# DHDev0/Stochastic-muzero

Measured on AMD Instinct MI355X. Metric: MCTS simulations/sec (whole node), CartPole MLP 4096 envs × 50 sims, higher is better.
Workload: dtype f32 (tree values, heads) + f64 (pUCT scores, root priors) + i32 (counts)

## Files before the change

### include/smz.h

```cpp
#ifndef SMZ_H
#define SMZ_H

#include <stddef.h>
#include <stdint.h>

#ifdef __cplusplus
extern "C" {
#endif

#define SMZ_ABI_VERSION 1
#define SMZ_MAX_ACTIONS 32
#define SMZ_MAX_ACTIONS_LARGE 1024
#define SMZ_MAX_PLAYER_CYCLE 32
#define SMZ_MT_WORDS 624

typedef enum {
    SMZ_OK = 0,
    SMZ_ERR_INVALID = -1,
    SMZ_ERR_HIP = -2,
    SMZ_ERR_NOMEM = -3,
    SMZ_ERR_STATE = -4,
    SMZ_ERR_TOO_LARGE = -5
} smz_status;

// ... 65 lines not shown

int smz_expand_backup_select(smz_handle *h, const float *hidden_dev, const float *reward_dev, const float *policy_dev,
                             const float *value_dev, float *parent_hidden_dev, int32_t *last_action_dev,
                             uint8_t *branch_dev, float *mlp_input_dev, smz_stream stream);

int smz_root_stats(smz_handle *h, int32_t *visits_dev, double *priors_dev, float *root_value_dev,
                   float *child_reward_dev, smz_stream stream);

int smz_act(smz_handle *h, double temperature, const double *pow_table_host, int32_t *action_dev, double *policy_dev,
            double *child_visits_dev, float *root_value_dev, smz_stream stream);

int smz_support_decode(const float *logits_dev, int S, float *out_dev, int B, smz_stream stream);
int smz_policy_softmax(const float *logits_dev, int A, float *out_dev, int B, smz_stream stream);
int smz_dynamics_epilogue(const float *state_dyn_dev, const float *state_after_dev, const float *reward_logits_dev,
                          int ld, const uint8_t *branch_dev, int S, float *hidden_out_dev, float *reward_out_dev, int B,
                          smz_stream stream);
int smz_prediction_epilogue(const float *policy_logits_pred_dev, const float *value_logits_pred_dev,
                            const float *policy_logits_after_dev, const float *value_logits_after_dev, int ld,
                            const uint8_t *branch_dev, int A, int S, float *policy_out_dev, float *value_out_dev,
                            int B, smz_stream stream);

typedef struct {
    int32_t obs, A, S, H, L;
    int32_t OP;
    int32_t total_floats;
    int32_t off[30];
} smz_mlp_desc;
int smz_mlp_layout(smz_mlp_desc *desc);
int smz_mlp_initial(const smz_mlp_desc *desc, const float *weights_dev, const float *obs_dev, float *hidden_out_dev,
                    float *policy_out_dev, int B, smz_stream stream);
int smz_mlp_recurrent(const smz_mlp_desc *desc, const float *weights_dev, const float *mlp_input_dev,
                      const uint8_t *branch_dev, float *hidden_out_dev, float *reward_out_dev, float *policy_out_dev,
                      float *value_out_dev, int B, smz_stream stream);

enum { SMZ_LSTM_TRUNKS = 7, SMZ_LSTM_MAX_LAYERS = 4, SMZ_LSTM_REP = 2 * SMZ_LSTM_TRUNKS * SMZ_LSTM_MAX_LAYERS,
       SMZ_LSTM_OFFSETS = SMZ_LSTM_REP + 2, SMZ_LSTM_SLACK = 256 };
typedef struct {
    int32_t obs, A, S, L;
    int32_t total_floats;
    int32_t recurrent_floats;
    int32_t lds_bytes;
    int32_t off[SMZ_LSTM_OFFSETS];
} smz_lstm_desc;
int smz_lstm_layout(smz_lstm_desc *desc);
int smz_lstm_initial(const smz_lstm_desc *desc, const float *weights_dev, const float *obs_dev, float *hidden_out_dev,
                     float *policy_out_dev, int B, smz_stream stream);
int smz_lstm_recurrent(const smz_lstm_desc *desc, const float *weights_dev, const float *mlp_input_dev,
                       const uint8_t *branch_dev, float *hidden_out_dev, float *reward_out_dev, float *policy_out_dev,
                       float *value_out_dev, int B, smz_stream stream);

enum { SMZ_V_DYN = 0, SMZ_V_ADY = 1, SMZ_V_PRE = 2, SMZ_V_APR = 3 };
enum { SMZ_VT_CONV_IN = 0, SMZ_VT_BN_IN, SMZ_VT_RES_A, SMZ_VT_RES_B, SMZ_VT_RES_BN, SMZ_VT_MIX_W, SMZ_VT_MIX_B,
       SMZ_VT_TOWER , SMZ_V_TRANS_STRIDE = 13 };
enum { SMZ_VP_RES_A = 0, SMZ_VP_RES_B, SMZ_VP_RES_BN, SMZ_VP_VMIX_W, SMZ_VP_VMIX_B, SMZ_VP_VTOWER ,
       SMZ_VP_PMIX_W = 11, SMZ_VP_PMIX_B, SMZ_VP_PTOWER , SMZ_V_PRED_STRIDE = 19 };
enum { SMZ_VR_STEM = 0, SMZ_VR_NARROW_A, SMZ_VR_NARROW_B, SMZ_VR_NARROW_BN, SMZ_VR_WIDEN, SMZ_VR_WIDE_A, SMZ_VR_WIDE_B,
       SMZ_VR_WIDE_BN, SMZ_VR_LAST_A, SMZ_VR_LAST_B, SMZ_VR_LAST_BN };
enum { SMZ_V_TRANS_BASE = 0, SMZ_V_PRED_BASE = 26, SMZ_V_REP_BASE = 64, SMZ_V_OFFSETS = 80 };
typedef struct smz_vision_desc {
    int32_t A, S, H, L;
    int32_t OP;
    int32_t total_floats;
    int32_t small_floats;
    int32_t off[SMZ_V_OFFSETS];
} smz_vision_desc;
int smz_vision_layout(smz_vision_desc *desc);
// ... 104 lines not shown
```

### stochastic-muzero_amd/_lib.py

```python
import ctypes as C
import os

_HERE = os.path.dirname(os.path.abspath(__file__))
LIB_PATH = os.environ.get("SMZ_LIB_PATH") or os.path.join(_HERE, "libsmz.so")

SMZ_OK, SMZ_ERR_INVALID, SMZ_ERR_HIP, SMZ_ERR_NOMEM, SMZ_ERR_STATE, SMZ_ERR_TOO_LARGE = 0, -1, -2, -3, -4, -5
RNG_MT19937_NUMPY, RNG_PHILOX = 0, 1
MAX_ACTIONS = 32
MAX_ACTIONS_LARGE = 1024


class SmzError(RuntimeError):
    def __init__(self, code, text):
        super().__init__(f"libsmz error {code}: {text}")
        self.code = code


class Config(C.Structure):
    _fields_ = [("num_trees", C.c_int32), ("num_actions", C.c_int32), ("max_action_sample", C.c_int32),
                ("hidden_size", C.c_int32), ("num_simulations", C.c_int32), ("pb_c_base", C.c_int32),
                ("pb_c_init", C.c_double), ("discount", C.c_double), ("root_dirichlet_alpha", C.c_double),
                ("root_exploration_fraction", C.c_double), ("rng_mode", C.c_int32), ("device", C.c_int32)]


# ... 30 lines not shown


_P = C.c_void_p
SIGNATURES = {
    "smz_create": (C.c_int, [C.POINTER(Config), C.POINTER(_P)]),
    "smz_create_large_actions": (C.c_int, [C.POINTER(Config), C.POINTER(_P)]),
    "smz_destroy": (C.c_int, [_P]),
    "smz_abi_version": (C.c_int, []),
    "smz_build_features": (C.c_int, []),
    "smz_last_error": (C.c_char_p, []),
    "smz_node_capacity": (C.c_int, [_P]),
    "smz_last_kernel": (C.c_int, [_P, C.c_char_p, C.c_int]),
    "smz_set_pb_c_table": (C.c_int, [_P, _P, C.c_int]),
    "smz_seed": (C.c_int, [_P, _P, _P]),
    "smz_set_rng_state": (C.c_int, [_P, C.c_int, _P, C.c_int]),
    "smz_get_rng_state": (C.c_int, [_P, C.c_int, _P, C.POINTER(C.c_int)]),
    "smz_philox_words": (C.c_int, [C.c_uint64, C.c_uint32, C.c_int, C.c_int, _P]),
    "smz_get_philox_position": (C.c_int, [_P, C.c_int, C.POINTER(C.c_uint32), C.POINTER(C.c_int)]),
    "smz_rng_snapshot": (C.c_int, [_P, _P]),
    "smz_rng_restore": (C.c_int, [_P, _P]),
    "smz_root_init": (C.c_int, [_P, _P, _P, _P, C.c_int, _P]),
    "smz_select": (C.c_int, [_P, _P, _P, _P, _P, _P]),
    "smz_expand_backup": (C.c_int, [_P, _P, _P, _P, _P, _P]),
    "smz_expand_backup_select": (C.c_int, [_P, _P, _P, _P, _P, _P, _P, _P, _P, _P]),
    "smz_root_stats": (C.c_int, [_P, _P, _P, _P, _P, _P]),
    "smz_act": (C.c_int, [_P, C.c_double, _P, _P, _P, _P, _P, _P]),
    "smz_support_decode": (C.c_int, [_P, C.c_int, _P, C.c_int, _P]),
    "smz_policy_softmax": (C.c_int, [_P, C.c_int, _P, C.c_int, _P]),
    "smz_dynamics_epilogue": (C.c_int, [_P, _P, _P, C.c_int, _P, C.c_int, _P, _P, C.c_int, _P]),
    "smz_prediction_epilogue": (C.c_int, [_P, _P, _P, _P, C.c_int, _P, C.c_int, C.c_int, _P, _P, C.c_int, _P]),
    "smz_mlp_layout": (C.c_int, [C.POINTER(MlpDesc)]),
    "smz_mlp_initial": (C.c_int, [C.POINTER(MlpDesc), _P, _P, _P, _P, C.c_int, _P]),
    "smz_mlp_recurrent": (C.c_int, [C.POINTER(MlpDesc), _P, _P, _P, _P, _P, _P, _P, C.c_int, _P]),
    "smz_mlp_layout_wide": (C.c_int, [C.POINTER(MlpDesc)]),
    "smz_mlp_recurrent_wide": (C.c_int, [C.POINTER(MlpDesc), _P, _P, _P, _P, _P, _P, _P, C.c_int, _P]),
    "smz_lstm_layout": (C.c_int, [C.POINTER(LstmDesc)]),
    "smz_lstm_initial": (C.c_int, [C.POINTER(LstmDesc), _P, _P, _P, _P, C.c_int, _P]),
    "smz_lstm_recurrent": (C.c_int, [C.POINTER(LstmDesc), _P, _P, _P, _P, _P, _P, _P, C.c_int, _P]),
    "smz_vision_layout": (C.c_int, [C.POINTER(VisionDesc)]),
    "smz_vision_initial": (C.c_int, [C.POINTER(VisionDesc), _P, _P, _P, _P, C.c_int, _P]),
    "smz_vision_initial_record": (C.c_int, [C.POINTER(VisionDesc), _P, _P, _P, _P, _P, C.c_int, _P]),
    "smz_vision_recurrent": (C.c_int, [C.POINTER(VisionDesc), _P, _P, C.c_int, _P, _P, _P, _P, _P, _P, C.c_int, _P]),
    "smz_search_mlp_act": (C.c_int, [_P, C.POINTER(MlpDesc), _P, _P, C.c_int, C.c_double, _P, _P, _P, _P, _P, _P]),
    "smz_search_mlp_act_cartpole": (C.c_int, [_P, C.POINTER(MlpDesc), _P, C.c_int, C.c_double, _P, _P, _P, _P, _P,
                                              C.POINTER(CartPoleEnv), _P]),
    "smz_search_mlp": (C.c_int, [_P, C.POINTER(MlpDesc), _P, _P, C.c_int, _P]),
    "smz_frames_resize_u8": (C.c_int, [_P, C.c_int, C.c_int, C.c_int, C.c_int, C.c_int, _P, _P, _P]),
    "smz_frames_resize_taps_u8": (C.c_int, [_P, C.c_int, C.c_int, C.c_int, C.c_int, C.c_int, _P, _P, _P]),
    "smz_host_register": (C.c_int, [_P, C.c_size_t]),
    "smz_host_unregister": (C.c_int, [_P]),
    "smz_copy_async": (C.c_int, [_P, _P, C.c_size_t, C.c_int, _P]),
    "smz_search_vision": (C.c_int, [_P, C.POINTER(VisionDesc), _P, _P, _P, C.c_int, _P]),
    "smz_search_vision_act": (C.c_int, [_P, C.POINTER(VisionDesc), _P, _P, _P, C.c_int, C.c_double, _P, _P, _P, _P, _P, _P]),
    "smz_cartpole_step": (C.c_int, [_P, _P, _P, _P, _P, C.c_int, _P]),
    "smz_cartpole_step_pack": (C.c_int, [_P, _P, _P, _P, _P, _P, C.c_int, C.c_int, _P, _P, _P, C.c_int, _P]),
    "smz_cartpole_step_ctl": (C.c_int, [_P, _P, _P, _P, _P, C.POINTER(EpisodeCtl), _P, C.c_int, C.c_int, _P, _P, _P, C.c_int, _P]),
    "smz_cartpole_reset_state": (C.c_int, [C.c_uint64, C.c_int64, C.c_int64, C.POINTER(C.c_double * 4)]),
    "smz_synthetic_obs": (C.c_int, [_P, C.c_int, C.c_int, C.c_uint64, C.c_int64, C.c_int64, _P]),
    "smz_set_active": (C.c_int, [_P, _P]),
    "smz_set_players": (C.c_int, [_P, C.c_int, _P, _P]),
    "smz_set_leaf_ids_out": (C.c_int, [_P, _P]),
    "smz_host_cartpole_step": (C.c_int, [_P, _P, _P, _P, _P, _P, C.c_int32, C.c_int]),
    "smz_get_hidden_layout": (C.c_int, [_P, C.POINTER(_P), C.POINTER(C.c_int), C.POINTER(C.c_int)]),
    "smz_mlp_recurrent_rows": (C.c_int, [C.POINTER(MlpDesc), _P, _P, C.c_int, C.c_int, _P, _P, _P, _P, _P, _P, C.c_int, _P]),
    "smz_traj_floats": (C.c_int, [C.c_int, C.c_int]),
    "smz_traj_pack": (C.c_int, [_P, C.c_int, C.c_int, C.c_int, C.c_int, _P, _P, _P, _P, _P, _P, _P, C.c_int, _P]),
# ... 55 lines not shown
```

### stochastic-muzero_amd/csrc/smz_mlp.hip

```cpp
#include <hip/hip_runtime.h>
#include <math.h>
#include <stdint.h>
#include <stdlib.h>
#include <stdio.h>

#include "../../include/smz.h"
#include "smz_mlp_device.hpp"

using namespace smz_mlp;

namespace {

extern __shared__ float4 smz_mlp_lds4[];

constexpr int kFastS = 31, kFastH = 64, kFastL = 0;
template <int U, bool FASTD>
__global__ void __launch_bounds__(512) k_mlp_recurrent(smz_mlp_desc d, const float *weights, const float *x,
                                                       const uint8_t *branch, float *hidden_out, float *reward_out,
                                                       float *policy_out, float *value_out, int B, int rows_per_wave) {
    float *lds = reinterpret_cast<float *>(smz_mlp_lds4);
    stage_recurrent_weights(lds, weights, d);
    if (FASTD) { d.S = kFastS; d.H = kFastH; d.L = kFastL; d.OP = kWave; }
    const int lane = threadIdx.x & (kWave - 1), wave = threadIdx.x / kWave, waves = blockDim.x / kWave;
    float *scratch = lds + d.total_floats + wave * scratch_floats(d);
    const int row0 = (blockIdx.x * waves + wave) * rows_per_wave;
    const int S = d.S, A = d.A, K4in = up4(S + A), rs = row_scratch_floats(d);
    for (int i = 0; i < rows_per_wave; i += kRows) {
        if (row0 + i >= B) break;
        const float *xin[kRows];
        bool dyn[kRows], live[kRows];
        float *dh[kRows], *dp[kRows];
        float reward[kRows], value[kRows];
#pragma unroll
        for (int r = 0; r < kRows; r++) {
            const int row = row0 + i + r;
            live[r] = (i + r < rows_per_wave) && row < B;
            const int rr = live[r] ? row : row0 + i;
            float *xb = scratch + r * rs;
            for (int k = lane; k < K4in; k += kWave) xb[k] = (k < S + A) ? x[(size_t)rr * (S + A) + k] : 0.f;
            xin[r] = xb;
            dyn[r] = branch[rr] != 0;
            dh[r] = hidden_out + (size_t)rr * S;
            dp[r] = policy_out + (size_t)rr * A;
        }
        lds_sync();
        recurrent_rows<U, kRows>(lds, d, scratch, xin, dyn, live, dh, dp, reward, value);
#pragma unroll
        for (int r = 0; r < kRows; r++) {
            if (live[r] && lane == 0) {
                if (reward_out) reward_out[row0 + i + r] = reward[r];
                value_out[row0 + i + r] = value[r];
            }
        }
    }
}

template <int U>
__global__ void __launch_bounds__(512) k_mlp_initial(smz_mlp_desc d, const float *weights, const float *obs,
                                                     float *hidden_out, float *policy_out, int B, int rows_per_wave) {
    float *lds = reinterpret_cast<float *>(smz_mlp_lds4);
    stage_initial_weights(lds, weights, d);
    const int wave = threadIdx.x / kWave, waves = blockDim.x / kWave;
    float *scratch = lds + d.total_floats + wave * scratch_floats(d);
    const int row0 = (blockIdx.x * waves + wave) * rows_per_wave;
    for (int i = 0; i < rows_per_wave; i++) {
        const int row = row0 + i;
        if (row >= B) break;
        initial_row<U>(lds, d, lds, d, scratch, obs + (size_t)row * d.obs, hidden_out + (size_t)row * d.S, nullptr,
                       policy_out + (size_t)row * d.A);
    }
}

typedef float v4f __attribute__((ext_vector_type(4)));
#ifndef SMZ_MFMA_COMPACT
#define SMZ_MFMA_COMPACT 1
#endif
constexpr bool kMfmaCompact = SMZ_MFMA_COMPACT != 0;
constexpr int kTileLeaves = 16, kMfmaWaves = kMfmaCompact ? 16 : 12;
constexpr int kTileFloats = 32 * 32;

__device__ inline float lane_xor16(float v) {
    const unsigned u = __float_as_uint(v);
    const auto r = __builtin_amdgcn_permlane16_swap(u, u, false, false);
    return __uint_as_float(((threadIdx.x & 16) ? r[0] : r[1]));
}
// ... 558 lines not shown
        const size_t lds2 = ((size_t)(kMfmaCompact ? compact_total_floats(*d) : d->total_floats - rep_floats(*d)) + (size_t)kMfmaWaves * kTileFloats) * sizeof(float) +
                            2 * kMaxChunk * sizeof(unsigned short) + 16;
        if (min_rows == 0 && lds2 > (size_t)kLdsBytes) return SMZ_ERR_TOO_LARGE;
        if (min_rows >= 0 && B >= min_rows && lds2 <= (size_t)kLdsBytes) {
            int chunk = mfma_chunk(B);
            int wgs = (B + chunk - 1) / chunk;
            if (wgs > 256) wgs = 256;
            if (d->A == 2) {
                if (allow_lds(k_mlp_recurrent_mfma<2, false>, lds2) != SMZ_OK) return SMZ_ERR_HIP;
                hipLaunchKernelGGL((k_mlp_recurrent_mfma<2, false>), dim3(wgs), dim3(kMfmaWaves * kWave), lds2, (hipStream_t)stream, *d, weights_dev,
                                   mlp_input_dev, branch_dev, hidden_out_dev, reward_out_dev, policy_out_dev, value_out_dev, B, chunk, TreeRows{});
            } else {
                if (allow_lds(k_mlp_recurrent_mfma<4, false>, lds2) != SMZ_OK) return SMZ_ERR_HIP;
                hipLaunchKernelGGL((k_mlp_recurrent_mfma<4, false>), dim3(wgs), dim3(kMfmaWaves * kWave), lds2, (hipStream_t)stream, *d, weights_dev,
                                   mlp_input_dev, branch_dev, hidden_out_dev, reward_out_dev, policy_out_dev, value_out_dev, B, chunk, TreeRows{});
            }
            return hipGetLastError() == hipSuccess ? SMZ_OK : SMZ_ERR_HIP;
        }
    }
    if (d->S == kFastS && d->H == kFastH && d->L == kFastL) {
        if (allow_lds(k_mlp_recurrent<1, true>, lds) != SMZ_OK) return SMZ_ERR_HIP;
        hipLaunchKernelGGL((k_mlp_recurrent<1, true>), dim3(blocks), dim3(kWavesPerWg * kWave), lds, (hipStream_t)stream, *d,
                           weights_dev, mlp_input_dev, branch_dev, hidden_out_dev, reward_out_dev, policy_out_dev,
                           value_out_dev, B, rpw);
    } else {
        if (allow_lds(k_mlp_recurrent<1, false>, lds) != SMZ_OK) return SMZ_ERR_HIP;
        hipLaunchKernelGGL((k_mlp_recurrent<1, false>), dim3(blocks), dim3(kWavesPerWg * kWave), lds, (hipStream_t)stream, *d,
                           weights_dev, mlp_input_dev, branch_dev, hidden_out_dev, reward_out_dev, policy_out_dev,
                           value_out_dev, B, rpw);
    }
    return hipGetLastError() == hipSuccess ? SMZ_OK : SMZ_ERR_HIP;
}

int smz_mlp_recurrent_rows(const smz_mlp_desc *d, const float *weights_dev, float *hidden_dev, int nodes_per_tree,
                           int row_stride, const int32_t *ids_dev, const int32_t *last_action_dev, const uint8_t *branch_dev,
                           float *reward_out_dev, float *policy_out_dev, float *value_out_dev, int B, smz_stream stream) {
    if (mlp_check(d, weights_dev) != SMZ_OK || !hidden_dev || !ids_dev || !last_action_dev || !branch_dev || !policy_out_dev ||
        !value_out_dev || B < 1 || nodes_per_tree < 1 || row_stride < d->S)
        return SMZ_ERR_INVALID;
    const int waves = mfma_launch_waves();
    const size_t lds2 = ((size_t)(kMfmaCompact ? compact_total_floats(*d) : d->total_floats - rep_floats(*d)) + (size_t)waves * kTileFloats) * sizeof(float) +
                        2 * kMaxChunk * sizeof(unsigned short) + 16;
    if (!(d->S == kFastS && d->H == kFastH && d->L == kFastL && (d->A == 2 || d->A == 4)) || lds2 > (size_t)kLdsBytes)
        return SMZ_ERR_TOO_LARGE;
    int chunk = mfma_chunk(B);
    int wgs = (B + chunk - 1) / chunk;
    if (wgs > 256) wgs = 256;
    const TreeRows tr = {hidden_dev, ids_dev, last_action_dev, nodes_per_tree, row_stride};
    if (d->A == 2) {
        if (allow_lds(k_mlp_recurrent_mfma<2, true>, lds2) != SMZ_OK) return SMZ_ERR_HIP;
        hipLaunchKernelGGL((k_mlp_recurrent_mfma<2, true>), dim3(wgs), dim3(waves * kWave), lds2, (hipStream_t)stream, *d, weights_dev,
                           nullptr, branch_dev, nullptr, reward_out_dev, policy_out_dev, value_out_dev, B, chunk, tr);
    } else {
        if (allow_lds(k_mlp_recurrent_mfma<4, true>, lds2) != SMZ_OK) return SMZ_ERR_HIP;
        hipLaunchKernelGGL((k_mlp_recurrent_mfma<4, true>), dim3(wgs), dim3(waves * kWave), lds2, (hipStream_t)stream, *d, weights_dev,
                           nullptr, branch_dev, nullptr, reward_out_dev, policy_out_dev, value_out_dev, B, chunk, tr);
    }
    return hipGetLastError() == hipSuccess ? SMZ_OK : SMZ_ERR_HIP;
}

int smz_mlp_layout_wide(smz_mlp_desc *d) {
    if (!d || d->obs < 1 || d->A < 1 || d->S < 1 || d->H < 1 || d->L < 0) return SMZ_ERR_INVALID;
    if (d->H > kWideOP || 2 * d->S > kWideOP || d->A + d->S > kWideOP) return SMZ_ERR_TOO_LARGE;
    d->OP = kWideOP;
    const int mid = d->L > 0 ? d->H : 0;
    const int K[M_COUNT] = {d->S + d->A, d->S + d->A, mid, mid, d->H, d->H, d->S, d->S, mid, mid, d->H, d->H, d->obs, mid, d->H};
// ... 32 lines not shown
```

### stochastic-muzero_amd/csrc/smz_mlp_device.hpp

```cpp
#pragma once
#include <hip/hip_runtime.h>
#include <math.h>
#include <stdint.h>

#include "../../include/smz.h"

namespace smz_mlp {

constexpr int kWave = 64;
enum { M_DYN_IN, M_ADY_IN, M_DYN_MID, M_ADY_MID, M_DYN_OUT, M_ADY_OUT, M_PRE_IN, M_APR_IN, M_PRE_MID, M_APR_MID,
       M_PRE_OUT, M_APR_OUT, M_REP_IN, M_REP_MID, M_REP_OUT, M_COUNT };

__host__ __device__ inline int up4(int x) { return (x + 3) & ~3; }

typedef float v2f __attribute__((ext_vector_type(2)));
__device__ inline v2f pk_fma(float wx, float wy, float ax, float ay, v2f c) {
    v2f w = {wx, wy}, a = {ax, ay};
    return __builtin_elementwise_fma(w, a, c);
}
template <int U, int R, bool SAME = false>
__device__ inline void dense(const float *const (&W)[R], const float *const (&bias)[R], const float *const (&act)[R], int K4,
                             const int (&OP)[R], int lane, float (&acc)[R][U]) {
    const float4 *a4[R], *w4[R];
    v2f acc2[R][U];
// ... 284 lines not shown
    for (int u = 0; u < U; u++) {
        const int o = lane + kWave * u;
        if (o < S) { const float e = smz_exp(v[u] - mr); den += e; num += (float)(o - half) * e; }
    }
    wave_sum2(den, num);
    float sc = mx - mn;
    if (sc < 1e-5f) sc += 1e-5f;
#pragma unroll
    for (int u = 0; u < U; u++) {
        const int o = lane + kWave * u;
        if (o >= S && o < 2 * S) {
            const float h = __fdividef(v[u] - mn, sc);
            act_out[o - S] = h;
            if (dst) dst[o - S] = h;
        }
    }
    return support_to_scalar(num, den);
}

__device__ inline void swap32(float &a, float &b) {
    const auto r = __builtin_amdgcn_permlane32_swap(__float_as_uint(a), __float_as_uint(b), false, false);
    a = __uint_as_float(r[0]);
    b = __uint_as_float(r[1]);
}
__device__ inline float half_bcast(float v, bool hi) {
    const float s0 = __int_as_float(__builtin_amdgcn_readlane(__float_as_int(v), 31));
    const float s1 = __int_as_float(__builtin_amdgcn_readlane(__float_as_int(v), 63));
    return hi ? s1 : s0;
}
#define SMZ_HSTEP1(I0, CTRL) I0 " %0, %0, %0 " CTRL "\n\t"
#define SMZ_HSTEP2(I0, I1, CTRL) I0 " %0, %0, %0 " CTRL "\n\t" I1 " %1, %1, %1 " CTRL "\n\t"
#define SMZ_HSTEP3(I0, I1, I2, CTRL) I0 " %0, %0, %0 " CTRL "\n\t" I1 " %1, %1, %1 " CTRL "\n\t" I2 " %2, %2, %2 " CTRL "\n\t"
#define SMZ_HSTEP5(I, CTRL) I " %0, %0, %0 " CTRL "\n\t" I " %1, %1, %1 " CTRL "\n\t" I " %2, %2, %2 " CTRL "\n\t" I " %3, %3, %3 " CTRL "\n\t" I " %4, %4, %4 " CTRL "\n\t"
#define SMZ_HALF_CHAIN(STEP, ...)                                                          \
    "s_nop 1\n\t" STEP(__VA_ARGS__, "row_shr:1 row_mask:0xf bank_mask:0xf") "s_nop 0\n\t"  \
    STEP(__VA_ARGS__, "row_shr:2 row_mask:0xf bank_mask:0xf") "s_nop 0\n\t"                \
    STEP(__VA_ARGS__, "row_shr:4 row_mask:0xf bank_mask:0xf") "s_nop 0\n\t"                \
    STEP(__VA_ARGS__, "row_shr:8 row_mask:0xf bank_mask:0xf") "s_nop 0\n\t"                \
    STEP(__VA_ARGS__, "row_bcast:15 row_mask:0xa bank_mask:0xf") "s_nop 1"
__device__ inline void half_max2(float &a, float &b) {
    asm SMZ_DPP_VOLATILE(SMZ_HALF_CHAIN(SMZ_HSTEP2, "v_max_f32_dpp", "v_max_f32_dpp") : "+v"(a), "+v"(b));
}
__device__ inline void half_minmax(float &mn, float &mx) {
    asm SMZ_DPP_VOLATILE(SMZ_HALF_CHAIN(SMZ_HSTEP2, "v_min_f32_dpp", "v_max_f32_dpp") : "+v"(mn), "+v"(mx));
}
__device__ inline void half_max_min_max(float &a, float &b, float &c) {
    asm SMZ_DPP_VOLATILE(SMZ_HALF_CHAIN(SMZ_HSTEP3, "v_max_f32_dpp", "v_min_f32_dpp", "v_max_f32_dpp") : "+v"(a), "+v"(b), "+v"(c));
}
__device__ inline void half_sum2(float &a, float &b) {
    asm SMZ_DPP_VOLATILE(SMZ_HALF_CHAIN(SMZ_HSTEP2, "v_add_f32_dpp", "v_add_f32_dpp") : "+v"(a), "+v"(b));
}
__device__ inline void half_sum3(float &a, float &b, float &c) {
    asm SMZ_DPP_VOLATILE(SMZ_HALF_CHAIN(SMZ_HSTEP3, "v_add_f32_dpp", "v_add_f32_dpp", "v_add_f32_dpp") : "+v"(a), "+v"(b), "+v"(c));
}
__device__ inline void half_sum5(float &a, float &b, float &c, float &d, float &e) {
    asm SMZ_DPP_VOLATILE(SMZ_HALF_CHAIN(SMZ_HSTEP5, "v_add_f32_dpp") : "+v"(a), "+v"(b), "+v"(c), "+v"(d), "+v"(e));
}

template <bool WITH_REWARD = false>
__device__ inline void softmax_decode_pair(float a0, float a1, int A, int S, int lane, float *dst0, float *dst1, float &val0,
                                           float &val1, float rnum = 0.f, float rden = 0.f, float *rew0 = nullptr, float *rew1 = nullptr) {
    float P = a0, Q = a1;
    swap32(P, Q);
    const bool hi = lane >= 32;
    const int j = lane & 31, oq = 32 + j, half = S / 2;
    const bool ppol = j < A, pval = !ppol && j < A + S, qval = oq >= A && oq < A + S;
    float mp = ppol ? P : -__builtin_inff();
    float mv = op_max(pval ? P : -__builtin_inff(), qval ? Q : -__builtin_inff());
    half_max2(mp, mv);
    mp = half_bcast(mp, hi); mv = half_bcast(mv, hi);
    const float eP = (ppol || pval) ? smz_exp(P - (ppol ? mp : mv)) : 0.f;
    const float eQ = qval ? smz_exp(Q - mv) : 0.f;
    float dp = ppol ? eP : 0.f, dvP = pval ? eP : 0.f, nvP = pval ? (float)(j - A - half) * eP : 0.f;
    float dv, nv;
    if (A + S == 33) {
        half_sum3(dp, dvP, nvP);
        int q = __builtin_amdgcn_update_dpp(0, __float_as_int(eQ), 0x140, 0xf, 0xf, false);
        q = __builtin_amdgcn_update_dpp(q, q, 0x142, 0xa, 0xf, false);
        const float e32 = __int_as_float(q);
        dv = dvP + e32;
        nv = nvP + (float)(32 - A - half) * e32;
    } else {
        float dvQ = eQ, nvQ = qval ? (float)(oq - A - half) * eQ : 0.f;
        half_sum5(dp, dvP, nvP, dvQ, nvQ);
        dv = dvP + dvQ; nv = nvP + nvQ;
    }
    if constexpr (WITH_REWARD) {
        const float sn = __int_as_float(__builtin_amdgcn_update_dpp(0, __float_as_int(rnum), 0x101, 0xf, 0xf, false));
        const float sd = __int_as_float(__builtin_amdgcn_update_dpp(0, __float_as_int(rden), 0x101, 0xf, 0xf, false));
        const bool rl = (lane & 31) == 30;
        nv = rl ? sn : nv;
        dv = rl ? sd : dv;
    }
    const float v = support_to_scalar(nv, dv);
    val0 = __int_as_float(__builtin_amdgcn_readlane(__float_as_int(v), 31));
    val1 = __int_as_float(__builtin_amdgcn_readlane(__float_as_int(v), 63));
    if constexpr (WITH_REWARD) {
        *rew0 = __int_as_float(__builtin_amdgcn_readlane(__float_as_int(v), 30));
        *rew1 = __int_as_float(__builtin_amdgcn_readlane(__float_as_int(v), 62));
    }
    const float dpb = half_bcast(dp, hi);
    float *dst = hi ? dst1 : dst0;
    if (ppol && dst) dst[j] = __fdividef(eP, dpb);
}

template <bool DEFER = false>
__device__ inline void dynamics_tail_pair(float a0, float a1, bool d0, bool d1, int S, int lane, float *act0, float *act1,
                                          float *dst0, float *dst1, float &rew0, float &rew1, float *rnum = nullptr, float *rden = nullptr) {
    float P = a0, Q = a1;
    swap32(P, Q);
    const bool hi = lane >= 32, dyn = hi ? d1 : d0;
    const int j = lane & 31, oq = 32 + j, half = S / 2;
    const bool plog = dyn && j < S;
    const bool pst = dyn ? j >= S : j < S, qst = dyn && oq < 2 * S;
    float mr = plog ? P : -__builtin_inff();
    float mn = op_min(pst ? P : __builtin_inff(), qst ? Q : __builtin_inff());
    float mx = op_max(pst ? P : -__builtin_inff(), qst ? Q : -__builtin_inff());
    half_max_min_max(mr, mn, mx);
    mr = half_bcast(mr, hi); mn = half_bcast(mn, hi); mx = half_bcast(mx, hi);
    const float e = plog ? smz_exp(P - mr) : 0.f;
    float den = e, num = plog ? (float)(j - half) * e : 0.f;
    half_sum2(den, num);
    if constexpr (DEFER) {
        *rnum = num; *rden = den;
        rew0 = rew1 = 0.f;
    } else {
        const float r = support_to_scalar(num, den);
        rew0 = d0 ? __int_as_float(__builtin_amdgcn_readlane(__float_as_int(r), 31)) : 0.f;
        rew1 = d1 ? __int_as_float(__builtin_amdgcn_readlane(__float_as_int(r), 63)) : 0.f;
    }
    float sc = mx - mn;
    if (sc < 1e-5f) sc += 1e-5f;
    float *act = hi ? act1 : act0, *dst = hi ? dst1 : dst0;
    const int ip = dyn ? j - S : j;
    if (pst) { const float h = __fdividef(P - mn, sc); act[ip] = h; if (dst) dst[ip] = h; }
    if (qst) { const float h = __fdividef(Q - mn, sc); act[oq - S] = h; if (dst) dst[oq - S] = h; }
}

template <bool PACKED = false>
__device__ inline void scale_pair(float a0, float a1, int S, int lane, float *act0, float *act1, float *dst0, float *dst1) {
    float P = a0, Q = a1;
    if (!PACKED) swap32(P, Q);
    const bool hi = lane >= 32;
    const int j = lane & 31;
    const bool in = j < S;
    float mn = in ? P : __builtin_inff(), mx = in ? P : -__builtin_inff();
    half_minmax(mn, mx);
    mn = half_bcast(mn, hi); mx = half_bcast(mx, hi);
    float sc = mx - mn;
    if (sc < 1e-5f) sc += 1e-5f;
    float *act = hi ? act1 : act0, *dst = hi ? dst1 : dst0;
    if (in) { const float h = __fdividef(P - mn, sc); act[j] = h; if (dst) dst[j] = h; }
}

struct MatOff {
    int w, b, op;
};
template <bool CP = false>
__device__ __host__ inline int mat_op(const smz_mlp_desc &d, int m) {
    if (!CP) return d.OP;
    const int o = (m == M_ADY_OUT) ? up4(d.S) : ((m == M_PRE_OUT || m == M_APR_OUT) ? up4(d.A + d.S) : ((m == M_DYN_OUT) ? up4(2 * d.S) : up4(d.H)));
    return o < d.OP ? o : d.OP;
}
template <bool CP = false>
__device__ __host__ inline int mat_off(const smz_mlp_desc &d, int m) {
    const int kin = up4(d.S + d.A), kmid = d.L > 0 ? up4(d.H) : 0, kh = up4(d.H), ks = up4(d.S), ko = up4(d.obs);
    const int K[M_COUNT] = {kin, kin, kmid, kmid, kh, kh, ks, ks, kmid, kmid, kh, kh, ko, kmid, kh};
    int floats = 0;
#pragma unroll
    for (int j = 0; j < M_COUNT; j++) floats += j < m ? K[j] * mat_op<CP>(d, j) : 0;
    return floats;
}
template <bool CP = false>
__device__ inline MatOff pick(const smz_mlp_desc &d, bool first, int ma, int mb) {
    MatOff o;
    const int bias0 = d.off[M_COUNT];
    o.w = first ? mat_off<CP>(d, ma) : mat_off<CP>(d, mb);
    o.b = bias0 + (first ? ma : mb) * d.OP;
    o.op = first ? mat_op<CP>(d, ma) : mat_op<CP>(d, mb);
    return o;
}
// ... 58 lines not shown

template <int U, int R, bool SAME = false, bool CP = false>
__device__ inline void recurrent_rows(const float *lds, const smz_mlp_desc &d, float *scratch, const float *const (&xin)[R],
                                      const bool (&dyn)[R], const bool (&live)[R], float *const (&dst_hidden)[R],
                                      float *const (&dst_policy)[R], float (&reward)[R], float (&value)[R]) {
    const int S = d.S, A = d.A, K4in = up4(S + A), K4h = up4(d.H), K4s = up4(S);
    const int lane = threadIdx.x & (kWave - 1);
    const int rs = row_scratch_floats(d), kin = rs - K4h - K4s;
    float *tA[R], *hbuf[R];
    MatOff m1[R], m1m[R], m3[R], m3m[R];
#pragma unroll
    for (int r = 0; r < R; r++) {
        tA[r] = scratch + r * rs + kin;
        hbuf[r] = tA[r] + K4h;
        m1[r] = pick<CP>(d, dyn[r], M_DYN_IN, M_ADY_IN);   m1m[r] = pick<CP>(d, dyn[r], M_DYN_MID, M_ADY_MID);
        m3[r] = pick<CP>(d, dyn[r], M_PRE_IN, M_APR_IN);   m3m[r] = pick<CP>(d, dyn[r], M_PRE_MID, M_APR_MID);
        for (int k = lane; k < K4s; k += kWave) hbuf[r][k] = 0.f;
    }
    trunk<U, R, SAME>(lds, d, m1, m1m, xin, K4in, tA, lane);
    float acc[R][U];
    constexpr bool PAIRED = SMZ_PAIR_TAILS && U == 1 && R == 2;
    const bool halves = PAIRED && SAME && SMZ_DENSE_HALVES && S <= 32 && !dyn[0] && !dyn[1];
    if (halves) {
        if constexpr (PAIRED && SAME) {
            const MatOff m = pick<CP>(d, false, M_DYN_OUT, M_ADY_OUT);
            acc[0][0] = dense_halves(lds + m.w, lds + m.b, tA[0], tA[1], K4h, m.op, lane);
            acc[1][0] = 0.f;
        }
    } else {
        const float *W[R], *Bv[R], *Ac[R];
        int op[R];
#pragma unroll
        for (int r = 0; r < R; r++) {
            const MatOff m = pick<CP>(d, dyn[r], M_DYN_OUT, M_ADY_OUT);
            W[r] = lds + m.w; Bv[r] = lds + m.b; Ac[r] = tA[r]; op[r] = m.op;
        }
        dense<U, R, SAME>(W, Bv, Ac, K4h, op, lane, acc);
    }
    float pair_rnum = 0.f, pair_rden = 0.f;
    bool pair_reward = false;
    if constexpr (PAIRED) {
        if (S <= 32) {
            reward[0] = reward[1] = 0.f;
            if (halves) scale_pair<true>(acc[0][0], 0.f, S, lane, hbuf[0], hbuf[1], live[0] ? dst_hidden[0] : nullptr,
                                         live[1] ? dst_hidden[1] : nullptr);
            else if (!dyn[0] && !dyn[1]) scale_pair(acc[0][0], acc[1][0], S, lane, hbuf[0], hbuf[1], live[0] ? dst_hidden[0] : nullptr,
                                               live[1] ? dst_hidden[1] : nullptr);
            else if (SMZ_ONE_DECODE) {
                dynamics_tail_pair<true>(acc[0][0], acc[1][0], dyn[0], dyn[1], S, lane, hbuf[0], hbuf[1], live[0] ? dst_hidden[0] : nullptr,
                                         live[1] ? dst_hidden[1] : nullptr, reward[0], reward[1], &pair_rnum, &pair_rden);
                pair_reward = true;
            } else dynamics_tail_pair(acc[0][0], acc[1][0], dyn[0], dyn[1], S, lane, hbuf[0], hbuf[1], live[0] ? dst_hidden[0] : nullptr,
                                      live[1] ? dst_hidden[1] : nullptr, reward[0], reward[1]);
        } else {
#pragma unroll
            for (int r = 0; r < R; r++) {
                reward[r] = 0.f;
                if (dyn[r]) reward[r] = decode_scale_lanes<U>(acc[r], S, lane, hbuf[r], live[r] ? dst_hidden[r] : nullptr);
                else scale_lanes<U>(acc[r], 0, S, lane, hbuf[r], live[r] ? dst_hidden[r] : nullptr);
            }
        }
    } else {
#pragma unroll
    for (int r = 0; r < R; r++) {
        reward[r] = 0.f;
        if (dyn[r]) {
            reward[r] = decode_scale_lanes<U>(acc[r], S, lane, hbuf[r], live[r] ? dst_hidden[r] : nullptr);
// ... 152 lines not shown
```

Before: 514.1 million.

## Add paired-row MLP recurrent kernel and half-wave allreduce via DPP butterfly

Adds a new recurrent kernel that processes two rows per wave and exposes it through the C API and Python bindings. It replaces the half-wave reduce-then-broadcast pattern with a butterfly allreduce built from DPP and permlane16_swap, which drops the separate broadcast step. It also folds the deferred reward sums into the existing policy/value reductions and merges the two conditional hidden stores into one. The pair kernel needs even B and callers must opt into it. The forced both_dyn pick looks odd and could select the wrong matrix when the rows differ.

```diff
diff --git a/include/smz.h b/include/smz.h
--- a/include/smz.h
+++ b/include/smz.h
@@ -121,6 +121,9 @@
 int smz_mlp_recurrent(const smz_mlp_desc *desc, const float *weights_dev, const float *mlp_input_dev,
                       const uint8_t *branch_dev, float *hidden_out_dev, float *reward_out_dev, float *policy_out_dev,
                       float *value_out_dev, int B, smz_stream stream);
+int smz_mlp_recurrent_pair(const smz_mlp_desc *desc, const float *weights_dev, const float *mlp_input_dev,
+                           const uint8_t *branch_dev, float *hidden_out_dev, float *reward_out_dev, float *policy_out_dev,
+                           float *value_out_dev, int B, smz_stream stream);
 
 enum { SMZ_LSTM_TRUNKS = 7, SMZ_LSTM_MAX_LAYERS = 4, SMZ_LSTM_REP = 2 * SMZ_LSTM_TRUNKS * SMZ_LSTM_MAX_LAYERS,
        SMZ_LSTM_OFFSETS = SMZ_LSTM_REP + 2, SMZ_LSTM_SLACK = 256 };
diff --git a/stochastic-muzero_amd/_lib.py b/stochastic-muzero_amd/_lib.py
--- a/stochastic-muzero_amd/_lib.py
+++ b/stochastic-muzero_amd/_lib.py
@@ -86,6 +86,7 @@
     "smz_mlp_layout": (C.c_int, [C.POINTER(MlpDesc)]),
     "smz_mlp_initial": (C.c_int, [C.POINTER(MlpDesc), _P, _P, _P, _P, C.c_int, _P]),
     "smz_mlp_recurrent": (C.c_int, [C.POINTER(MlpDesc), _P, _P, _P, _P, _P, _P, _P, C.c_int, _P]),
+    "smz_mlp_recurrent_pair": (C.c_int, [C.POINTER(MlpDesc), _P, _P, _P, _P, _P, _P, _P, C.c_int, _P]),
     "smz_mlp_layout_wide": (C.c_int, [C.POINTER(MlpDesc)]),
     "smz_mlp_recurrent_wide": (C.c_int, [C.POINTER(MlpDesc), _P, _P, _P, _P, _P, _P, _P, C.c_int, _P]),
     "smz_lstm_layout": (C.c_int, [C.POINTER(LstmDesc)]),
diff --git a/stochastic-muzero_amd/csrc/smz_mlp.hip b/stochastic-muzero_amd/csrc/smz_mlp.hip
--- a/stochastic-muzero_amd/csrc/smz_mlp.hip
+++ b/stochastic-muzero_amd/csrc/smz_mlp.hip
@@ -51,6 +51,44 @@
                 if (reward_out) reward_out[row0 + i + r] = reward[r];
                 value_out[row0 + i + r] = value[r];
             }
+        }
+    }
+}
+
+template <bool FASTD>
+__global__ void __launch_bounds__(512) k_mlp_recurrent_pair(smz_mlp_desc d, const float *weights, const float *x,
+                                                            const uint8_t *branch, float *hidden_out, float *reward_out,
+                                                            float *policy_out, float *value_out, int B, int pairs_per_wave) {
+    float *lds = reinterpret_cast<float *>(smz_mlp_lds4);
+    stage_recurrent_weights(lds, weights, d);
+    if (FASTD) { d.S = kFastS; d.H = kFastH; d.L = kFastL; d.OP = kWave; }
+    const int lane = threadIdx.x & (kWave - 1), wave = threadIdx.x / kWave, waves = blockDim.x / kWave;
+    const int S = d.S, A = d.A, K4in = up4(S + A), rs = row_scratch_floats(d);
+    float *scratch = lds + d.total_floats + wave * 2 * rs;
+    const int pair0 = (blockIdx.x * waves + wave) * pairs_per_wave;
+    for (int i = 0; i < pairs_per_wave; i++) {
+        const int row = 2 * (pair0 + i);
+        if (row + 1 >= B) break;
+        const float *xin[2];
+        bool dyn[2];
+        const bool live[2] = {true, true};
+        float *dh[2], *dp[2];
+        float reward[2], value[2];
+#pragma unroll
+        for (int r = 0; r < 2; r++) {
+            float *xb = scratch + r * rs;
+            for (int k = lane; k < K4in; k += kWave) xb[k] = (k < S + A) ? x[(size_t)(row + r) * (S + A) + k] : 0.f;
+            xin[r] = xb;
+            dyn[r] = branch[row + r] != 0;
+            dh[r] = hidden_out + (size_t)(row + r) * S;
+            dp[r] = policy_out + (size_t)(row + r) * A;
+        }
+        lds_sync();
+        if (dyn[0] == dyn[1]) recurrent_rows<1, 2, true>(lds, d, scratch, xin, dyn, live, dh, dp, reward, value);
+        else recurrent_rows<1, 2, false>(lds, d, scratch, xin, dyn, live, dh, dp, reward, value);
+        if (lane < 2) {
+            if (reward_out) reward_out[row + lane] = lane ? reward[1] : reward[0];
+            value_out[row + lane] = lane ? value[1] : value[0];
         }
     }
 }
@@ -675,6 +713,31 @@
     return hipGetLastError() == hipSuccess ? SMZ_OK : SMZ_ERR_HIP;
 }
 
+int smz_mlp_recurrent_pair(const smz_mlp_desc *d, const float *weights_dev, const float *mlp_input_dev,
+                           const uint8_t *branch_dev, float *hidden_out_dev, float *reward_out_dev, float *policy_out_dev,
+                           float *value_out_dev, int B, smz_stream stream) {
+    if (mlp_check(d, weights_dev) != SMZ_OK || !mlp_input_dev || !branch_dev || !hidden_out_dev || !policy_out_dev ||
+        !value_out_dev || B < 2 || (B & 1))
+        return SMZ_ERR_INVALID;
+    const int pairs = B / 2;
+    int ppw = (pairs + 256 * kWavesPerWg - 1) / (256 * kWavesPerWg);
+    const int blocks = (pairs + ppw * kWavesPerWg - 1) / (ppw * kWavesPerWg);
+    const size_t lds = ((size_t)d->total_floats + (size_t)kWavesPerWg * 2 * row_scratch_floats(*d)) * sizeof(float);
+    if (lds > (size_t)kLdsBytes) return SMZ_ERR_TOO_LARGE;
+    if (d->S == kFastS && d->H == kFastH && d->L == kFastL) {
+        if (allow_lds(k_mlp_recurrent_pair<true>, lds) != SMZ_OK) return SMZ_ERR_HIP;
+        hipLaunchKernelGGL((k_mlp_recurrent_pair<true>), dim3(blocks), dim3(kWavesPerWg * kWave), lds, (hipStream_t)stream, *d,
+                           weights_dev, mlp_input_dev, branch_dev, hidden_out_dev, reward_out_dev, policy_out_dev,
+                           value_out_dev, B, ppw);
+    } else {
+        if (allow_lds(k_mlp_recurrent_pair<false>, lds) != SMZ_OK) return SMZ_ERR_HIP;
+        hipLaunchKernelGGL((k_mlp_recurrent_pair<false>), dim3(blocks), dim3(kWavesPerWg * kWave), lds, (hipStream_t)stream, *d,
+                           weights_dev, mlp_input_dev, branch_dev, hidden_out_dev, reward_out_dev, policy_out_dev,
+                           value_out_dev, B, ppw);
+    }
+    return hipGetLastError() == hipSuccess ? SMZ_OK : SMZ_ERR_HIP;
+}
+
 int smz_mlp_recurrent_rows(const smz_mlp_desc *d, const float *weights_dev, float *hidden_dev, int nodes_per_tree,
                            int row_stride, const int32_t *ids_dev, const int32_t *last_action_dev, const uint8_t *branch_dev,
                            float *reward_out_dev, float *policy_out_dev, float *value_out_dev, int B, smz_stream stream) {
diff --git a/stochastic-muzero_amd/csrc/smz_mlp_device.hpp b/stochastic-muzero_amd/csrc/smz_mlp_device.hpp
--- a/stochastic-muzero_amd/csrc/smz_mlp_device.hpp
+++ b/stochastic-muzero_amd/csrc/smz_mlp_device.hpp
@@ -340,29 +340,67 @@
 #define SMZ_HSTEP2(I0, I1, CTRL) I0 " %0, %0, %0 " CTRL "\n\t" I1 " %1, %1, %1 " CTRL "\n\t"
 #define SMZ_HSTEP3(I0, I1, I2, CTRL) I0 " %0, %0, %0 " CTRL "\n\t" I1 " %1, %1, %1 " CTRL "\n\t" I2 " %2, %2, %2 " CTRL "\n\t"
 #define SMZ_HSTEP5(I, CTRL) I " %0, %0, %0 " CTRL "\n\t" I " %1, %1, %1 " CTRL "\n\t" I " %2, %2, %2 " CTRL "\n\t" I " %3, %3, %3 " CTRL "\n\t" I " %4, %4, %4 " CTRL "\n\t"
-#define SMZ_HALF_CHAIN(STEP, ...)                                                          \
-    "s_nop 1\n\t" STEP(__VA_ARGS__, "row_shr:1 row_mask:0xf bank_mask:0xf") "s_nop 0\n\t"  \
-    STEP(__VA_ARGS__, "row_shr:2 row_mask:0xf bank_mask:0xf") "s_nop 0\n\t"                \
-    STEP(__VA_ARGS__, "row_shr:4 row_mask:0xf bank_mask:0xf") "s_nop 0\n\t"                \
-    STEP(__VA_ARGS__, "row_shr:8 row_mask:0xf bank_mask:0xf") "s_nop 0\n\t"                \
+#define SMZ_HSTEP7(I, CTRL) SMZ_HSTEP5(I, CTRL) I " %5, %5, %5 " CTRL "\n\t" I " %6, %6, %6 " CTRL "\n\t"
+#define SMZ_HALF_CHAIN(PAD, STEP, ...)                                                     \
+    "s_nop 1\n\t" STEP(__VA_ARGS__, "row_shr:1 row_mask:0xf bank_mask:0xf") PAD            \
+    STEP(__VA_ARGS__, "row_shr:2 row_mask:0xf bank_mask:0xf") PAD                          \
+    STEP(__VA_ARGS__, "row_shr:4 row_mask:0xf bank_mask:0xf") PAD                          \
+    STEP(__VA_ARGS__, "row_shr:8 row_mask:0xf bank_mask:0xf") PAD                          \
     STEP(__VA_ARGS__, "row_bcast:15 row_mask:0xa bank_mask:0xf") "s_nop 1"
+#define SMZ_PAD2 "s_nop 0\n\t"
 __device__ inline void half_max2(float &a, float &b) {
-    asm SMZ_DPP_VOLATILE(SMZ_HALF_CHAIN(SMZ_HSTEP2, "v_max_f32_dpp", "v_max_f32_dpp") : "+v"(a), "+v"(b));
+    asm SMZ_DPP_VOLATILE(SMZ_HALF_CHAIN(SMZ_PAD2, SMZ_HSTEP2, "v_max_f32_dpp", "v_max_f32_dpp") : "+v"(a), "+v"(b));
 }
 __device__ inline void half_minmax(float &mn, float &mx) {
-    asm SMZ_DPP_VOLATILE(SMZ_HALF_CHAIN(SMZ_HSTEP2, "v_min_f32_dpp", "v_max_f32_dpp") : "+v"(mn), "+v"(mx));
+    asm SMZ_DPP_VOLATILE(SMZ_HALF_CHAIN(SMZ_PAD2, SMZ_HSTEP2, "v_min_f32_dpp", "v_max_f32_dpp") : "+v"(mn), "+v"(mx));
 }
 __device__ inline void half_max_min_max(float &a, float &b, float &c) {
-    asm SMZ_DPP_VOLATILE(SMZ_HALF_CHAIN(SMZ_HSTEP3, "v_max_f32_dpp", "v_min_f32_dpp", "v_max_f32_dpp") : "+v"(a), "+v"(b), "+v"(c));
+    asm SMZ_DPP_VOLATILE(SMZ_HALF_CHAIN("", SMZ_HSTEP3, "v_max_f32_dpp", "v_min_f32_dpp", "v_max_f32_dpp") : "+v"(a), "+v"(b), "+v"(c));
 }
 __device__ inline void half_sum2(float &a, float &b) {
-    asm SMZ_DPP_VOLATILE(SMZ_HALF_CHAIN(SMZ_HSTEP2, "v_add_f32_dpp", "v_add_f32_dpp") : "+v"(a), "+v"(b));
+    asm SMZ_DPP_VOLATILE(SMZ_HALF_CHAIN(SMZ_PAD2, SMZ_HSTEP2, "v_add_f32_dpp", "v_add_f32_dpp") : "+v"(a), "+v"(b));
 }
 __device__ inline void half_sum3(float &a, float &b, float &c) {
-    asm SMZ_DPP_VOLATILE(SMZ_HALF_CHAIN(SMZ_HSTEP3, "v_add_f32_dpp", "v_add_f32_dpp", "v_add_f32_dpp") : "+v"(a), "+v"(b), "+v"(c));
+    asm SMZ_DPP_VOLATILE(SMZ_HALF_CHAIN("", SMZ_HSTEP3, "v_add_f32_dpp", "v_add_f32_dpp", "v_add_f32_dpp") : "+v"(a), "+v"(b), "+v"(c));
 }
 __device__ inline void half_sum5(float &a, float &b, float &c, float &d, float &e) {
-    asm SMZ_DPP_VOLATILE(SMZ_HALF_CHAIN(SMZ_HSTEP5, "v_add_f32_dpp") : "+v"(a), "+v"(b), "+v"(c), "+v"(d), "+v"(e));
+    asm SMZ_DPP_VOLATILE(SMZ_HALF_CHAIN("", SMZ_HSTEP5, "v_add_f32_dpp") : "+v"(a), "+v"(b), "+v"(c), "+v"(d), "+v"(e));
+}
+__device__ inline void half_sum7(float &a, float &b, float &c, float &d, float &e, float &f, float &g) {
+    asm SMZ_DPP_VOLATILE(SMZ_HALF_CHAIN("", SMZ_HSTEP7, "v_add_f32_dpp") : "+v"(a), "+v"(b), "+v"(c), "+v"(d), "+v"(e), "+v"(f), "+v"(g));
+}
+
+#ifndef SMZ_HALF_ALLREDUCE
+#define SMZ_HALF_ALLREDUCE 1
+#endif
+#define SMZ_ROW_BUTTERFLY(PAD, STEP, ...)                                                  \
+    "s_nop 1\n\t" STEP(__VA_ARGS__, "quad_perm:[1,0,3,2] row_mask:0xf bank_mask:0xf") PAD  \
+    STEP(__VA_ARGS__, "quad_perm:[2,3,0,1] row_mask:0xf bank_mask:0xf") PAD                \
+    STEP(__VA_ARGS__, "row_half_mirror row_mask:0xf bank_mask:0xf") PAD                    \
+    STEP(__VA_ARGS__, "row_mirror row_mask:0xf bank_mask:0xf") "s_nop 1"
+__device__ inline void rows_even_odd(float v, float &even, float &odd) {
+    const auto r = __builtin_amdgcn_permlane16_swap(__float_as_uint(v), __float_as_uint(v), false, false);
+    even = __uint_as_float(r[0]);
+    odd = __uint_as_float(r[1]);
+}
+__device__ inline void half_all_minmax(float &mn, float &mx) {
+    asm SMZ_DPP_VOLATILE(SMZ_ROW_BUTTERFLY(SMZ_PAD2, SMZ_HSTEP2, "v_min_f32_dpp", "v_max_f32_dpp") : "+v"(mn), "+v"(mx));
+    float a0, a1, b0, b1;
+    rows_even_odd(mn, a0, a1); rows_even_odd(mx, b0, b1);
+    asm SMZ_DPP_VOLATILE("s_nop 1\n\tv_min_f32 %0, %2, %3\n\tv_max_f32 %1, %4, %5" : "=&v"(mn), "=&v"(mx) : "v"(a0), "v"(a1), "v"(b0), "v"(b1));
+}
+__device__ inline void half_all_max2(float &a, float &b) {
+    asm SMZ_DPP_VOLATILE(SMZ_ROW_BUTTERFLY(SMZ_PAD2, SMZ_HSTEP2, "v_max_f32_dpp", "v_max_f32_dpp") : "+v"(a), "+v"(b));
+    float a0, a1, b0, b1;
+    rows_even_odd(a, a0, a1); rows_even_odd(b, b0, b1);
+    asm SMZ_DPP_VOLATILE("s_nop 1\n\tv_max_f32 %0, %2, %3\n\tv_max_f32 %1, %4, %5" : "=&v"(a), "=&v"(b) : "v"(a0), "v"(a1), "v"(b0), "v"(b1));
+}
+__device__ inline void half_all_max_min_max(float &a, float &b, float &c) {
+    asm SMZ_DPP_VOLATILE(SMZ_ROW_BUTTERFLY("", SMZ_HSTEP3, "v_max_f32_dpp", "v_min_f32_dpp", "v_max_f32_dpp") : "+v"(a), "+v"(b), "+v"(c));
+    float a0, a1, b0, b1, c0, c1;
+    rows_even_odd(a, a0, a1); rows_even_odd(b, b0, b1); rows_even_odd(c, c0, c1);
+    asm SMZ_DPP_VOLATILE("s_nop 1\n\tv_max_f32 %0, %3, %4\n\tv_min_f32 %1, %5, %6\n\tv_max_f32 %2, %7, %8"
+                         : "=&v"(a), "=&v"(b), "=&v"(c) : "v"(a0), "v"(a1), "v"(b0), "v"(b1), "v"(c0), "v"(c1));
 }
 
 template <bool WITH_REWARD = false>
@@ -375,14 +413,19 @@
     const bool ppol = j < A, pval = !ppol && j < A + S, qval = oq >= A && oq < A + S;
     float mp = ppol ? P : -__builtin_inff();
     float mv = op_max(pval ? P : -__builtin_inff(), qval ? Q : -__builtin_inff());
+#if SMZ_HALF_ALLREDUCE
+    half_all_max2(mp, mv);
+#else
     half_max2(mp, mv);
     mp = half_bcast(mp, hi); mv = half_bcast(mv, hi);
+#endif
     const float eP = (ppol || pval) ? smz_exp(P - (ppol ? mp : mv)) : 0.f;
     const float eQ = qval ? smz_exp(Q - mv) : 0.f;
     float dp = ppol ? eP : 0.f, dvP = pval ? eP : 0.f, nvP = pval ? (float)(j - A - half) * eP : 0.f;
     float dv, nv;
     if (A + S == 33) {
-        half_sum3(dp, dvP, nvP);
+        if constexpr (WITH_REWARD) half_sum5(dp, dvP, nvP, rnum, rden);
+        else half_sum3(dp, dvP, nvP);
         int q = __builtin_amdgcn_update_dpp(0, __float_as_int(eQ), 0x140, 0xf, 0xf, false);
         q = __builtin_amdgcn_update_dpp(q, q, 0x142, 0xa, 0xf, false);
         const float e32 = __int_as_float(q);
@@ -390,7 +433,8 @@
         nv = nvP + (float)(32 - A - half) * e32;
     } else {
         float dvQ = eQ, nvQ = qval ? (float)(oq - A - half) * eQ : 0.f;
-        half_sum5(dp, dvP, nvP, dvQ, nvQ);
+        if constexpr (WITH_REWARD) half_sum7(dp, dvP, nvP, dvQ, nvQ, rnum, rden);
+        else half_sum5(dp, dvP, nvP, dvQ, nvQ);
         dv = dvP + dvQ; nv = nvP + nvQ;
     }
     if constexpr (WITH_REWARD) {
@@ -424,15 +468,19 @@
     float mr = plog ? P : -__builtin_inff();
     float mn = op_min(pst ? P : __builtin_inff(), qst ? Q : __builtin_inff());
     float mx = op_max(pst ? P : -__builtin_inff(), qst ? Q : -__builtin_inff());
+#if SMZ_HALF_ALLREDUCE
+    half_all_max_min_max(mr, mn, mx);
+#else
     half_max_min_max(mr, mn, mx);
     mr = half_bcast(mr, hi); mn = half_bcast(mn, hi); mx = half_bcast(mx, hi);
+#endif
     const float e = plog ? smz_exp(P - mr) : 0.f;
     float den = e, num = plog ? (float)(j - half) * e : 0.f;
-    half_sum2(den, num);
     if constexpr (DEFER) {
         *rnum = num; *rden = den;
         rew0 = rew1 = 0.f;
     } else {
+        half_sum2(den, num);
         const float r = support_to_scalar(num, den);
         rew0 = d0 ? __int_as_float(__builtin_amdgcn_readlane(__float_as_int(r), 31)) : 0.f;
         rew1 = d1 ? __int_as_float(__builtin_amdgcn_readlane(__float_as_int(r), 63)) : 0.f;
@@ -440,9 +488,8 @@
     float sc = mx - mn;
     if (sc < 1e-5f) sc += 1e-5f;
     float *act = hi ? act1 : act0, *dst = hi ? dst1 : dst0;
-    const int ip = dyn ? j - S : j;
-    if (pst) { const float h = __fdividef(P - mn, sc); act[ip] = h; if (dst) dst[ip] = h; }
-    if (qst) { const float h = __fdividef(Q - mn, sc); act[oq - S] = h; if (dst) dst[oq - S] = h; }
+    const int ix = pst ? (dyn ? j - S : j) : oq - S;
+    if (pst || qst) { const float h = __fdividef((pst ? P : Q) - mn, sc); act[ix] = h; if (dst) dst[ix] = h; }
 }
 
 template <bool PACKED = false>
@@ -453,8 +500,12 @@
     const int j = lane & 31;
     const bool in = j < S;
     float mn = in ? P : __builtin_inff(), mx = in ? P : -__builtin_inff();
+#if SMZ_HALF_ALLREDUCE
+    half_all_minmax(mn, mx);
+#else
     half_minmax(mn, mx);
     mn = half_bcast(mn, hi); mx = half_bcast(mx, hi);
+#endif
     float sc = mx - mn;
     if (sc < 1e-5f) sc += 1e-5f;
     float *act = hi ? act1 : act0, *dst = hi ? dst1 : dst0;
@@ -579,7 +630,8 @@
         int op[R];
 #pragma unroll
         for (int r = 0; r < R; r++) {
-            const MatOff m = pick<CP>(d, dyn[r], M_DYN_OUT, M_ADY_OUT);
+            const bool both_dyn = PAIRED && SAME && SMZ_DENSE_HALVES && S <= 32;
+            const MatOff m = pick<CP>(d, both_dyn ? true : dyn[r], M_DYN_OUT, M_ADY_OUT);
             W[r] = lds + m.w; Bv[r] = lds + m.b; Ac[r] = tA[r]; op[r] = m.op;
         }
         dense<U, R, SAME>(W, Bv, Ac, K4h, op, lane, acc);
```

Result: slower. 484.3 million (-5.8%).
